# treangenlab/Seqwin

Measured on AMD Instinct MI355X. Metric: Gbp/s minimizer-indexed, higher is better.
Workload: dtype u64

## Files before the change

### seqwin_amd/csrc/radix.hip

```cpp
#include <algorithm>
#include <cstdlib>
#include <cstring>
#include <vector>
#include <map>
#include <mutex>

#include "device.hpp"

namespace sw {
namespace {

constexpr int RS_ITEMS = 16;
#ifdef SW_RS_STAMPS
__device__ unsigned long long *g_rs_stamps = nullptr;
#define RS_STAMP(i)                                                                                        \
    do {                                                                                                   \
        if (g_rs_stamps && (tile & 63u) == 0 && threadIdx.x == 0) g_rs_stamps[(size_t)(tile >> 6) * 16 + (i)] = clock64(); \
    } while (0)
#else
#define RS_STAMP(i) do { } while (0)
#endif
#ifndef RS_LOOK
#define RS_LOOK 4
#endif
// ... 920 lines not shown
            unsigned long long *ptr = stamps.p;
            SW_HIP(hipMemcpyToSymbolAsync(HIP_SYMBOL(g_rs_stamps), &ptr, sizeof ptr, 0, hipMemcpyHostToDevice, stream));
        }
#endif
        unsigned long long *cur = perm_hi32 && p == 0 ? cursor.p : nullptr;
        hipLaunchKernelGGL(k_rs_scan<BITS>, dim3(1), dim3(RADIX), 0, stream, hist.p + (size_t)p * RADIX, cur);
        const uint32_t epoch = cur ? 0u : next_epoch(su.b, stream);
        auto launch = [&](auto kern) {
            hipLaunchKernelGGL(kern, dim3((unsigned)std::min<uint64_t>(n_tiles, (uint64_t)grid_p)), dim3(THREADS), 0, stream, keys, alt, n,
                               (uint32_t)n_tiles, sh, bits, hist.p + (size_t)p * RADIX, su.b.p, tickets.p + p, d_fail, dbg, cur,
                               RS_CURSOR_STRIDE, 64u, epoch);
        };
        if (cur ? !ballot_forced() : atomic_rank) launch(k_rs_pass_p<THREADS, BITS, 1>);
        else launch(k_rs_pass_p<THREADS, BITS, 0>);
        SW_HIP(hipGetLastError());
#ifdef SW_RS_STAMPS
        if (stamps.p) {
            std::vector<unsigned long long> hs(n_st);
            SW_HIP(hipStreamSynchronize(stream));
            SW_HIP(hipMemcpy(hs.data(), stamps.p, stamps.bytes(), hipMemcpyDeviceToHost));
            double acc[8] = {0}, look[3] = {0};
            size_t cnt = 0;
            for (size_t t = 0; t + 16 <= n_st; t += 16) {
                if (!hs[t] || !hs[t + 7]) continue;
                for (int i = 1; i <= 7; ++i) acc[i] += (double)(hs[t + i] - hs[t + i - 1]);
                for (int i = 0; i < 3; ++i) look[i] += (double)hs[t + 8 + i];
                ++cnt;
            }
            static const char *nm[] = {"", "rank", "barrier", "totals+scan", "barrier+scatter", "lookback(d0)", "barrier", "write-out"};
            fprintf(stderr, "[rs stamps] %d x %d bits, pass %u, %zu tiles sampled; mean clocks:", THREADS, BITS, p, cnt);
            double sum = 0;
            for (int i = 1; i <= 7; ++i) { fprintf(stderr, " %s=%.0f", nm[i], cnt ? acc[i] / cnt : 0.0); sum += cnt ? acc[i] / cnt : 0.0; }
            fprintf(stderr, " | tile %.0f | look-back of digit 0: %.1f steps, %.1f polls of an unpublished record, %.1f records behind\n", sum,
                    cnt ? look[0] / cnt : 0.0, cnt ? look[1] / cnt : 0.0, cnt ? look[2] / cnt : 0.0);
        }
#endif
        std::swap(keys, alt);
    }
}

}

namespace {
__global__ void k_rs_perm_cursors(unsigned long long *__restrict__ cursor, uint32_t n_groups, uint32_t radix, uint32_t stride,
                                  unsigned group_bits, unsigned digit_shift)
{
    const uint32_t i = blockIdx.x * blockDim.x + threadIdx.x;
    if (i >= n_groups * radix) return;
    const uint64_t g = i / radix, d = i % radix;
    cursor[(size_t)i * stride] = (group_bits < 64 ? g << group_bits : 0ull) + (d << digit_shift);
}
}

bool radix_unsort_perm_begin(UnsortPerm &u, uint64_t n, unsigned low_bits, unsigned nbit, hipStream_t stream)
{
    constexpr int THREADS = 512, BITS = 8;
    constexpr uint32_t RADIX = 1u << BITS, TILE = THREADS * RS_ITEMS;
    static_assert(UNSORT_CURSOR_STRIDE == RS_CURSOR_STRIDE, "one cursor layout for the first pass and for a producer that scatters itself");
    if (n == 0 || nbit <= low_bits + 8 || nbit > low_bits + 16) return false;
    if ((1ull << (low_bits + 8)) % TILE) return false;
    u.low_bits = low_bits;
    u.hi_bits = nbit - low_bits - 8;
    u.n_groups = (uint32_t)((n + (1ull << (low_bits + 8)) - 1) >> (low_bits + 8));
    const uint64_t n_tiles = (n + TILE - 1) / TILE;
    u.n_tiles = (uint32_t)n_tiles;
    int dev = 0, per_cu = 0;
    SW_HIP(hipGetDevice(&dev));
    hipDeviceProp_t prop;
    SW_HIP(hipGetDeviceProperties(&prop, dev));
    SW_HIP(hipOccupancyMaxActiveBlocksPerMultiprocessor(&per_cu, k_rs_pass_p<THREADS, BITS, 0>, THREADS, 0));
    u.grid = (unsigned)std::min<uint64_t>(n_tiles, (uint64_t)std::max(1, per_cu) * std::max(1, prop.multiProcessorCount));
    if (!u.cur_a.p) {
        u.cur_a.alloc((size_t)RADIX * RS_CURSOR_STRIDE);
        u.cur_b.alloc((size_t)u.n_groups * RADIX);
        u.tickets.alloc(2);
    }
    SW_HIP(hipMemsetAsync(u.tickets.p, 0, 8, stream));
    hipLaunchKernelGGL(k_rs_perm_cursors, dim3(1), dim3(RADIX), 0, stream, u.cur_a.p, 1u, RADIX, RS_CURSOR_STRIDE, 64u, low_bits + 8);
    hipLaunchKernelGGL(k_rs_perm_cursors, dim3((u.n_groups * RADIX + 255) / 256), dim3(256), 0, stream, u.cur_b.p, u.n_groups, RADIX, 1u,
                       low_bits + 8, low_bits);
    SW_HIP(hipGetLastError());
    return true;
}

void radix_unsort_perm_first(UnsortPerm &u, const uint64_t *keys, uint64_t *alt, uint64_t n, hipStream_t stream, uint32_t *d_fail)
{
    constexpr int THREADS = 512, BITS = 8;
    auto pass = ballot_forced() ? k_rs_pass_p<THREADS, BITS, 0> : k_rs_pass_p<THREADS, BITS, 1>;
    hipLaunchKernelGGL(pass, dim3(u.grid), dim3(THREADS), 0, stream, keys, alt, n, u.n_tiles, 32u + u.low_bits + 8, u.hi_bits,
                       (const unsigned long long *)nullptr, (unsigned long long *)nullptr, u.tickets.p, d_fail, 0u, u.cur_a.p,
                       RS_CURSOR_STRIDE, 64u, 0u);
    SW_HIP(hipGetLastError());
}

void radix_unsort_perm_second(UnsortPerm &u, const uint64_t *keys, uint64_t *alt, uint64_t n, hipStream_t stream, uint32_t *d_fail)
{
    constexpr int THREADS = 512, BITS = 8;
    auto pass = ballot_forced() ? k_rs_pass_p<THREADS, BITS, 0> : k_rs_pass_p<THREADS, BITS, 1>;
    hipLaunchKernelGGL(pass, dim3(u.grid), dim3(THREADS), 0, stream, keys, alt, n, u.n_tiles, 32u + u.low_bits, 8u,
                       (const unsigned long long *)nullptr, (unsigned long long *)nullptr, u.tickets.p + 1, d_fail, 0u, u.cur_b.p, 1u,
                       u.low_bits + 8, 0u);
    SW_HIP(hipGetLastError());
}

bool radix_unsort_perm(uint64_t *&keys, uint64_t *&alt, uint64_t n, unsigned low_bits, unsigned nbit, hipStream_t stream, uint32_t *d_fail)
{
    UnsortPerm u;
    if (!radix_unsort_perm_begin(u, n, low_bits, nbit, stream)) return false;
    radix_unsort_perm_first(u, keys, alt, n, stream, d_fail);
    std::swap(keys, alt);
    radix_unsort_perm_second(u, keys, alt, n, stream, d_fail);
    std::swap(keys, alt);
    return true;
}

bool radix_pairs_available() { return rank_mode() == 1; }
int radix_rank_mode() { return rank_mode(); }

uint64_t radix_trim_state()
{
    uint64_t freed = 0;
    if (g_state_uses) return 0;
    std::lock_guard<std::mutex> lock(state_registry_mu());
    for (auto &kv : state_registry()) {
        StateBuf &b = *kv.second;
        std::unique_lock<std::mutex> use(b.mu, std::try_to_lock);
        if (!use.owns_lock() || !b.p) continue;
        int cur = -1;
        (void)hipGetDevice(&cur);
        if (cur != kv.first.first) (void)hipSetDevice(kv.first.first);
        (void)hipFree(b.p);
        if (cur != kv.first.first && cur >= 0) (void)hipSetDevice(cur);
        freed += b.words * 8;
        b.p = nullptr;
        b.words = 0;
        b.epoch = 0;
    }
    return freed;
}

void radix_demote_rank()
{
    int dev = 0;
    SW_HIP(hipGetDevice(&dev));
    std::lock_guard<std::mutex> lock(rank_mu());
    rank_modes()[dev] = 0;
}

void radix_sort_pairs32(uint32_t *&keys, uint32_t *&keys_alt, OccPay *&vals, OccPay *&vals_alt, uint64_t n, unsigned end_bit,
                        hipStream_t stream, uint32_t *d_fail, const StageSource *src, const std::function<void()> &after_first,
                        uint32_t *low_out)
{
    constexpr uint32_t RADIX = 1u << RP_BITS, TILE = RP_THREADS * RP_ITEMS;
    if (n == 0 || end_bit == 0) return;
    if (end_bit > 32 || end_bit % RP_BITS) raise(SW_ERR_RUNTIME, "radix_sort_pairs32: key bits must be a multiple of 8 up to 32");
    if (n >= 0xFFFFFFFFull) raise(SW_ERR_RUNTIME, "radix_sort_pairs32: more than 2^32-2 elements");
    const unsigned n_passes = end_bit / RP_BITS;
    const uint64_t n_tiles = (n + TILE - 1) / TILE;
    int grid_p = 0;
    {
        static std::mutex &mu = *new std::mutex;
        static std::map<int, int> &grids = *new std::map<int, int>;
        int dev = 0;
        SW_HIP(hipGetDevice(&dev));
        std::lock_guard<std::mutex> lock(mu);
        int &g = grids[dev];
        if (!g) {
            int per_cu = 0;
            hipDeviceProp_t prop;
            SW_HIP(hipGetDeviceProperties(&prop, dev));
            SW_HIP(hipOccupancyMaxActiveBlocksPerMultiprocessor(&per_cu, k_rs_pair_pass<0>, RP_THREADS, 0));
            g = std::max(1, per_cu) * std::max(1, prop.multiProcessorCount);
        }
        grid_p = g;
    }
    DevArray<unsigned long long> hist((size_t)n_passes * RADIX);
    DevArray<uint32_t> tickets(n_passes);
    SW_HIP(hipMemsetAsync(tickets.p, 0, tickets.bytes(), stream));
    SW_HIP(hipMemsetAsync(hist.p, 0, hist.bytes(), stream));
    StageSource stage{};
    DevArray<uint32_t> chunk_tile;
    DevArray<unsigned long long> chunk_dir;
    if (src && src->rows) {
        stage = *src;
        hipLaunchKernelGGL(k_rs_hist32_rows, dim3((unsigned)((n + 16383) / 16384)), dim3(256), 0, stream,
                           reinterpret_cast<const uint4 *>(src->rows), n, n_passes, hist.p);
    } else if (src) {
        constexpr uint64_t CHUNK = 64 * RP_ITEMS;
        static_assert(TILE == (RP_THREADS / 64) * CHUNK, "a tile is one chunk per wave");
        const uint64_t n_chunks = (n + CHUNK - 1) / CHUNK;
        stage = *src;
        chunk_tile.alloc(n_chunks);
        chunk_dir.alloc(n_chunks * STAGE_ROW);
        stage.chunk_dir = chunk_dir.p;
        hipLaunchKernelGGL(k_rs_chunk_tiles, dim3((stage.n_tiles + 255u) / 256u), dim3(256), 0, stream, stage.tile_count, stage.dst_off,
                           stage.n_tiles, chunk_tile.p);
        hipLaunchKernelGGL(k_rs_stage_prepare, dim3((unsigned)std::min<uint64_t>(2048, (n_chunks + 3) / 4)), dim3(256), 0, stream, stage,
                           (const uint32_t *)chunk_tile.p, n, n_passes, chunk_dir.p, hist.p);
    } else {
        hipLaunchKernelGGL(k_rs_hist32, dim3((unsigned)((n + 65535) / 65536)), dim3(256), 0, stream, keys, n, n_passes, hist.p);
    }
    SW_HIP(hipGetLastError());
    StateUse su = state_buf(stream, (size_t)n_tiles * RADIX);
    StateBuf &sb = su.b;
    const StageSource none{};
    const uint32_t fault = fault_rank();
    for (unsigned p = 0; p < n_passes; ++p) {
        hipLaunchKernelGGL(k_rs_scan<RP_BITS>, dim3(1), dim3(RADIX), 0, stream, hist.p + (size_t)p * RADIX, (unsigned long long *)nullptr);
        const uint32_t epoch = next_epoch(sb, stream);
        const dim3 grid((unsigned)std::min<uint64_t>(n_tiles, (uint64_t)grid_p));
        if (p == 0 && src) {
            auto first = src->rows ? k_rs_pair_pass<2> : k_rs_pair_pass<1>;
            hipLaunchKernelGGL(first, grid, dim3(RP_THREADS), 0, stream, (const uint32_t *)nullptr, (const uint4 *)nullptr,
                               keys_alt, reinterpret_cast<uint4 *>(vals_alt), n, (uint32_t)n_tiles, 0u,
                               (const unsigned long long *)hist.p, sb.p, epoch, tickets.p, d_fail, stage,
                               n_passes == 1 ? low_out : (uint32_t *)nullptr, fault);
            SW_HIP(hipGetLastError());
            if (after_first) after_first();
        } else {
            hipLaunchKernelGGL(k_rs_pair_pass<0>, grid, dim3(RP_THREADS), 0, stream, (const uint32_t *)keys,
                               reinterpret_cast<const uint4 *>(vals), keys_alt, reinterpret_cast<uint4 *>(vals_alt), n, (uint32_t)n_tiles,
                               RP_BITS * p, (const unsigned long long *)(hist.p + (size_t)p * RADIX), sb.p, epoch, tickets.p + p, d_fail,
                               none, p + 1 == n_passes ? low_out : (uint32_t *)nullptr, fault);
            SW_HIP(hipGetLastError());
        }
        std::swap(keys, keys_alt);
        std::swap(vals, vals_alt);
    }
}

namespace {
constexpr uint32_t EB_RADIX = 512, EB_TABLE = EB_RADIX * EB_RADIX, EB_THREADS = 512;
constexpr uint64_t EB_EMPTY = ~0ull;
static_assert(EB_THREADS == EB_RADIX, "k_eb_finish: one bin per thread");
enum : uint32_t { EB_F_OVERFLOW = 1u, EB_F_RANGE = 2u, EB_F_ORDER = 4u };
struct EbInfo {
    unsigned long long n_sentinels;
    uint32_t n_tiles2, max_bucket, flags, n_runs, n_live, pad;
};

__global__ __launch_bounds__(EB_RADIX) void k_eb_level1(const unsigned long long *__restrict__ h1, uint32_t tile_keys,
                                                        unsigned long long *__restrict__ cursor, unsigned long long *__restrict__ segtab,
                                                        EbInfo *__restrict__ info)
{
    __shared__ unsigned long long s[EB_RADIX];
    __shared__ uint32_t st[EB_RADIX];
    const uint32_t d = threadIdx.x;
    const unsigned long long c = h1[d];
    const uint32_t tiles = (uint32_t)((c + tile_keys - 1) / tile_keys);
    s[d] = c;
    st[d] = tiles;
    __syncthreads();
    for (uint32_t o = 1; o < EB_RADIX; o <<= 1) {
        const unsigned long long a = d >= o ? s[d - o] : 0;
        const uint32_t b = d >= o ? st[d - o] : 0;
        __syncthreads();
        s[d] += a;
        st[d] += b;
        __syncthreads();
    }
    const unsigned long long first = s[d] - c;
    cursor[(size_t)d * RS_CURSOR_STRIDE] = first;
    uint32_t w = st[d] - tiles;
    for (uint32_t t = 0; t < tiles; ++t)
        segtab[w + t] = seg_pack(first + (uint64_t)t * tile_keys, d, (uint32_t)min((unsigned long long)tile_keys, c - (uint64_t)t * tile_keys));
    if (d == EB_RADIX - 1) info->n_tiles2 = st[d];
}

__global__ __launch_bounds__(1024) void k_eb_count(const uint64_t *__restrict__ in, const unsigned long long *__restrict__ segtab,
                                                   const EbInfo *__restrict__ info, unsigned shift, uint32_t dmask, uint64_t sentinel,
                                                   uint32_t *__restrict__ table, EbInfo *__restrict__ out)
{
    __shared__ uint32_t hist[EB_RADIX];
    __shared__ uint32_t s_sent;
    const uint32_t n_tiles = info->n_tiles2;
    for (uint32_t w = blockIdx.x; w < n_tiles; w += gridDim.x) {
        const unsigned long long seg = segtab[w];
        const uint64_t first = seg_first(seg);
        const uint32_t cnt = seg_count(seg);
        if (threadIdx.x < EB_RADIX) hist[threadIdx.x] = 0;
        if (threadIdx.x == 0) s_sent = 0;
        __syncthreads();
        uint64_t key[RS_ITEMS];
#pragma unroll
        for (int i = 0; i < RS_ITEMS; ++i) {
            const uint32_t li = i * 1024 + threadIdx.x;
            key[i] = li < cnt ? in[first + li] : EB_EMPTY;
        }
        uint32_t sent = 0;
#pragma unroll
        for (int i = 0; i < RS_ITEMS; ++i) {
            if (key[i] == EB_EMPTY) continue;
            if (key[i] == sentinel) ++sent;
            atomicAdd(&hist[(uint32_t)(key[i] >> shift) & dmask], 1u);
        }
        if (sent) atomicAdd(&s_sent, sent);
        __syncthreads();
        if (threadIdx.x < EB_RADIX && hist[threadIdx.x]) atomicAdd(&table[seg_bucket(seg) * EB_RADIX + threadIdx.x], hist[threadIdx.x]);
        if (threadIdx.x == 0 && s_sent) atomicAdd(&out->n_sentinels, (unsigned long long)s_sent);
        __syncthreads();
    }
}

__global__ __launch_bounds__(1024) void k_eb_scan(const uint32_t *__restrict__ cnt, const unsigned long long *__restrict__ n_sent,
                                                  uint32_t sent_at, uint32_t *__restrict__ start, unsigned long long *__restrict__ cursor,
                                                  uint32_t *__restrict__ max_out, uint32_t *__restrict__ total_out,
                                                  uint4 *__restrict__ live, uint32_t *__restrict__ n_live_out)
{
    constexpr uint32_t PER4 = EB_TABLE / 1024 / 4;
    __shared__ uint32_t ws[16], wm[16], wz[16];
    const uint32_t tid = threadIdx.x, lane = tid & 63u, wave = tid >> 6;
    const uint32_t sent = n_sent ? (uint32_t)*n_sent : 0u;
    const uint4 *cnt4 = reinterpret_cast<const uint4 *>(cnt) + (size_t)tid * PER4;
    uint32_t sum = 0, mx = 0, nz = 0;
#pragma unroll 16
    for (uint32_t j = 0; j < PER4; ++j) {
        const uint4 c = cnt4[j];
        mx = max(max(max(mx, c.x), max(c.y, c.z)), c.w);
        sum += c.x + c.y + c.z + c.w;
        nz += (c.x != 0) + (c.y != 0) + (c.z != 0) + (c.w != 0);
    }
    if (n_sent && sent_at / (4 * PER4) == tid) {
        mx = 0;
        for (uint32_t j = 0; j < 4 * PER4; ++j) {
            const uint32_t i = tid * 4 * PER4 + j, c = cnt[i];
            mx = max(mx, c - (i == sent_at ? min(c, sent) : 0u));
        }
    }
    uint32_t incl = sum, inz = nz;
    for (uint32_t o = 1; o < 64; o <<= 1) {
        const uint32_t up = __shfl_up(incl, o, 64), uz = __shfl_up(inz, o, 64);
        if (lane >= o) {
            incl += up;
            inz += uz;
        }
        mx = max(mx, __shfl_xor(mx, o, 64));
    }
    if (lane == 63) {
        ws[wave] = incl;
        wz[wave] = inz;
    }
    if (lane == 0) wm[wave] = mx;
    __syncthreads();
    uint32_t run = incl - sum, below = inz - nz, n_live = 0;
    for (uint32_t w = 0; w < 16; ++w) {
        if (w < wave) {
            run += ws[w];
            below += wz[w];
        }
        n_live += wz[w];
    }
    uint32_t at = n_live - 1u - below;
    uint4 *start4 = reinterpret_cast<uint4 *>(start) + (size_t)tid * PER4;
    ulonglong2 *cur2 = reinterpret_cast<ulonglong2 *>(cursor) + (size_t)tid * PER4 * 2;
#pragma unroll 16
    for (uint32_t j = 0; j < PER4; ++j) {
        const uint4 c = cnt4[j];
        const uint4 st = make_uint4(run, run + c.x, run + c.x + c.y, run + c.x + c.y + c.z);
        start4[j] = st;
        if (cursor) {
            cur2[2 * j] = make_ulonglong2(st.x, st.y);
            cur2[2 * j + 1] = make_ulonglong2(st.z, st.w);
        }
        if (live) {
            const uint32_t id = (tid * PER4 + j) * 4;
            if (c.x) live[at--] = make_uint4(id, st.x, c.x, 0u);
            if (c.y) live[at--] = make_uint4(id + 1, st.y, c.y, 0u);
            if (c.z) live[at--] = make_uint4(id + 2, st.z, c.z, 0u);
            if (c.w) live[at--] = make_uint4(id + 3, st.w, c.w, 0u);
        }
        run = st.w + c.w;
    }
    if (tid == 1023) {
        start[EB_TABLE] = run;
        if (total_out) *total_out = run;
        if (n_live_out) *n_live_out = n_live;
        uint32_t m = 0;
        for (uint32_t w = 0; w < 16; ++w) m = max(m, wm[w]);
        if (max_out) *max_out = m;
    }
}

#ifdef SW_RS_STAMPS
__device__ unsigned long long *g_eb_stamps = nullptr;
constexpr uint32_t EB_ST_EVERY = 16, EB_ST_WORDS = 16;
#define EB_STAMP(i) do { if (st) st[i] = clock64(); } while (0)
#define EB_STAMP_ADD(i, since) do { if (st) { const unsigned long long t_ = clock64(); st[i] += t_ - (since); (since) = t_; } } while (0)
#else
#define EB_STAMP(i) do { } while (0)
#define EB_STAMP_ADD(i, since) do { } while (0)
#endif

template <bool PACKED>
__global__ __launch_bounds__(EB_THREADS) void k_eb_finish(const uint64_t *__restrict__ in, const uint4 *__restrict__ live, uint32_t slots,
                                                          unsigned shift1, unsigned shift2, uint32_t mask2, unsigned bin_shift,
                                                          uint32_t bin_mask, unsigned cb, uint64_t sentinel,
                                                          uint64_t *__restrict__ tk, uint32_t *__restrict__ tc,
                                                          uint32_t *__restrict__ n_distinct, uint32_t *__restrict__ flags)
{
    extern __shared__ __align__(16) unsigned char eb_lds[];
    unsigned long long *hk = reinterpret_cast<unsigned long long *>(eb_lds);
    uint32_t *hc = reinterpret_cast<uint32_t *>(hk + slots);
    uint16_t *idx = PACKED ? reinterpret_cast<uint16_t *>(hk + slots) : reinterpret_cast<uint16_t *>(hc + slots);
    __shared__ uint32_t bd[EB_RADIX + 1], bk[EB_RADIX], bcur[EB_RADIX], wsd[EB_THREADS / 64], wsk[EB_THREADS / 64];
    __shared__ uint32_t s_over;
    const uint32_t tid = threadIdx.x, lane = tid & 63u, wave = tid >> 6;
#ifdef SW_RS_STAMPS
    unsigned long long *st = g_eb_stamps && tid == 0 && blockIdx.x % EB_ST_EVERY == 0 ? g_eb_stamps + (size_t)(blockIdx.x / EB_ST_EVERY) * EB_ST_WORDS : nullptr;
    unsigned long long st_t = 0;
#endif
    EB_STAMP(0);
    const uint4 me = live[blockIdx.x];
    const uint32_t mask = slots - 1u;
    for (uint32_t s = tid; s < slots; s += EB_THREADS) {
        hk[s] = EB_EMPTY;
        if (!PACKED) hc[s] = 0;
    }
    bd[tid] = 0;
    bk[tid] = 0;
    if (tid == 0) s_over = 0;
    const uint32_t b = me.x, first = me.y, cnt = me.z;
    const uint64_t low_mask = (1ull << shift2) - 1ull, count_mask = (1ull << cb) - 1ull;
    const uint64_t high = ((uint64_t)(b / EB_RADIX) << shift1) | ((uint64_t)(b % EB_RADIX) << shift2);
    uint64_t nxt[4];
#pragma unroll
    for (int i = 0; i < 4; ++i) {
        const uint32_t j = i * EB_THREADS + tid;
        nxt[i] = j < cnt ? in[(uint64_t)first + j] : sentinel;
    }
    EB_STAMP(1);
    __syncthreads();
    EB_STAMP(2);
#ifdef SW_RS_STAMPS
    if (st) st_t = clock64();
#endif
    uint32_t bad = 0;
    for (uint32_t j0 = 0; j0 < cnt; j0 += 4 * EB_THREADS) {
        if (*(volatile uint32_t *)&s_over) break;
        uint64_t key[4];
#pragma unroll
        for (int i = 0; i < 4; ++i) key[i] = nxt[i];
        if (j0 + 4 * EB_THREADS < cnt) {
#pragma unroll
            for (int i = 0; i < 4; ++i) {
                const uint32_t j = j0 + 4 * EB_THREADS + i * EB_THREADS + tid;
                nxt[i] = j < cnt ? in[(uint64_t)first + j] : sentinel;
            }
        }
        uint32_t cp[4], h[4];
        unsigned long long w[4];
#pragma unroll
        for (int i = 0; i < 4; ++i) {
            const uint64_t k = key[i];
            bool alive = k != sentinel;
            if (alive && ((uint32_t)(k >> shift1) * EB_RADIX + ((uint32_t)(k >> shift2) & mask2)) != b) {
                bad = 1;
                alive = false;
            }
            uint32_t copies = 1;
            const uint64_t any = __ballot(alive);
            if (any) {
                const int src = __ffsll((long long)any) - 1;
                const uint64_t k0 = (uint64_t)__shfl((unsigned long long)k, src, 64);
                const uint64_t same = __ballot(alive && k == k0);
                if (alive && k == k0) {
                    copies = (uint32_t)__popcll(same);
                    alive = (int)lane == src;
                }
            }
            cp[i] = alive ? copies : 0u;
            h[i] = (uint32_t)((k * 0x9E3779B97F4A7C15ull) >> 40) & mask;
            w[i] = PACKED ? ((k & low_mask) << cb) | copies : (unsigned long long)k;
        }
        EB_STAMP_ADD(3, st_t);
        for (uint32_t probes = 0; cp[0] | cp[1] | cp[2] | cp[3]; ++probes) {
            if (probes == slots) {
                s_over = 1;
                break;
            }
            unsigned long long old[4];
#pragma unroll
            for (int i = 0; i < 4; ++i)
                if (cp[i]) old[i] = atomicCAS(&hk[h[i]], EB_EMPTY, w[i]);
#pragma unroll
            for (int i = 0; i < 4; ++i) {
                if (!cp[i]) continue;
                if (PACKED) {
                    if (old[i] == EB_EMPTY) cp[i] = 0;
                    else if ((old[i] >> cb) == (w[i] >> cb)) {
                        atomicAdd(&hk[h[i]], (unsigned long long)cp[i]);
                        cp[i] = 0;
                    } else h[i] = (h[i] + 1u) & mask;
                } else {
                    if (old[i] == EB_EMPTY || old[i] == w[i]) {
                        atomicAdd(&hc[h[i]], cp[i]);
                        cp[i] = 0;
                    } else h[i] = (h[i] + 1u) & mask;
                }
            }
        }
        EB_STAMP_ADD(4, st_t);
    }
    if (bad) atomicOr(flags, EB_F_RANGE);
    __syncthreads();
    EB_STAMP(5);
    if (s_over) {
        if (tid == 0) atomicOr(flags, EB_F_OVERFLOW);
        return;
    }
    const unsigned wbin_shift = PACKED ? bin_shift + cb : bin_shift;
    for (uint32_t s = tid; s < slots; s += EB_THREADS) {
        const uint64_t k = hk[s];
        if (k == EB_EMPTY) continue;
        const uint32_t bin = (uint32_t)(k >> wbin_shift) & bin_mask;
        atomicAdd(&bd[bin], 1u);
        atomicAdd(&bk[bin], PACKED ? (uint32_t)(k & count_mask) : hc[s]);
    }
    __syncthreads();
    EB_STAMP(6);
    {
        const uint32_t d = bd[tid], c = bk[tid];
        uint32_t id = d, ic = c;
        for (uint32_t o = 1; o < 64; o <<= 1) {
            const uint32_t ud = __shfl_up(id, o, 64), uc = __shfl_up(ic, o, 64);
            if (lane >= o) {
                id += ud;
                ic += uc;
            }
        }
        if (lane == 63) {
            wsd[wave] = id;
            wsk[wave] = ic;
        }
        __syncthreads();
        uint32_t pd = id - d, pc = ic - c;
        for (uint32_t w2 = 0; w2 < wave; ++w2) {
            pd += wsd[w2];
            pc += wsk[w2];
        }
        bd[tid] = pd;
        bcur[tid] = pd;
        bk[tid] = pc;
        if (tid == EB_THREADS - 1) bd[EB_RADIX] = pd + d;
    }
    __syncthreads();
    EB_STAMP(7);
    for (uint32_t s = tid; s < slots; s += EB_THREADS) {
        const uint64_t k = hk[s];
        if (k == EB_EMPTY) continue;
        idx[atomicAdd(&bcur[(uint32_t)(k >> wbin_shift) & bin_mask], 1u)] = (uint16_t)s;
    }
    __syncthreads();
    EB_STAMP(8);
    const uint32_t n_dist = bd[EB_RADIX];
    if (tid == 0) n_distinct[b] = n_dist;
    for (uint32_t j = tid; j < n_dist; j += EB_THREADS) {
        const uint32_t s = idx[j];
        const uint64_t k = hk[s];
        const uint32_t bin = (uint32_t)(k >> wbin_shift) & bin_mask, lo = bd[bin], hi = bd[bin + 1];
        uint32_t less = 0, copies_less = 0;
        for (uint32_t i = lo; i < hi; i += 4) {
            uint32_t s2[4];
            unsigned long long k2[4];
            uint32_t c2[4];
#pragma unroll
            for (int u = 0; u < 4; ++u) s2[u] = i + u < hi ? idx[i + u] : s;
#pragma unroll
            for (int u = 0; u < 4; ++u) {
                k2[u] = hk[s2[u]];
                c2[u] = PACKED ? 0u : hc[s2[u]];
            }
#pragma unroll
            for (int u = 0; u < 4; ++u) {
                if (PACKED ? (k2[u] >> cb) < (k >> cb) : k2[u] < k) {
                    ++less;
                    copies_less += PACKED ? (uint32_t)(k2[u] & count_mask) : c2[u];
                }
            }
        }
        tk[(uint64_t)first + lo + less] = PACKED ? high | (k >> cb) : k;
        tc[(uint64_t)first + lo + less] = first + bk[bin] + copies_less;
    }
#ifdef SW_RS_STAMPS
    if (st) {
        st[9] = clock64();
        st[10] = cnt;
        st[11] = n_dist;
    }
#endif
}

__global__ __launch_bounds__(256) void k_eb_compact(const uint64_t *__restrict__ tk, const uint32_t *__restrict__ tc,
                                                    const uint4 *__restrict__ live, uint32_t n_live, const uint32_t *__restrict__ start,
                                                    const uint32_t *__restrict__ dstart,
                                                    const unsigned long long *__restrict__ n_sentinels, uint64_t *__restrict__ ukeys,
                                                    uint32_t *__restrict__ ucnt, uint32_t *__restrict__ flags)
{
    if (blockIdx.x == 0 && threadIdx.x == 0) ucnt[dstart[EB_TABLE]] = start[EB_TABLE] - (uint32_t)*n_sentinels;
    if (blockIdx.x >= n_live) return;
    const uint4 me = live[blockIdx.x];
    const uint32_t b = me.x, d0 = dstart[b], n = dstart[b + 1] - d0;
    if (n == 0) return;
    const uint64_t first = me.y;
    const uint32_t end = me.y + me.z;
    uint32_t bad = 0;
    for (uint32_t j = threadIdx.x; j < n; j += 256) {
        const uint64_t k = tk[first + j];
        const uint32_t c = tc[first + j];
        if (j + 1 < n && (tk[first + j + 1] <= k || tc[first + j + 1] <= c)) bad = 1;
        if (c < first || c >= end) bad = 1;
        ukeys[d0 + j] = k;
        ucnt[d0 + j] = c;
    }
    if (bad) atomicOr(flags, EB_F_ORDER);
}
}

int radix_edge_buckets(uint64_t *&keys, uint64_t *&alt, uint64_t m, unsigned key_bits, uint64_t sentinel,
                       const unsigned long long *d_hist_top, uint32_t cap, uint32_t slots, uint64_t *ukeys, uint32_t *ucnt,
                       uint32_t *n_runs, hipStream_t stream, uint32_t *d_fail, bool debug)
{
    constexpr int THREADS = 1024, BITS = 9;
    constexpr uint32_t TILE = THREADS * RS_ITEMS;
    unsigned digit_bits = 0, n_passes = 0;
    radix_layout(key_bits, &digit_bits, &n_passes);
    if (n_passes < 2 || m >= (1ull << 32) - 1 || slots < 64 || slots > 8192 || (slots & (slots - 1))) return 1;
    const unsigned shift1 = (n_passes - 1) * digit_bits, bits1 = key_bits - shift1;
    const unsigned bits2 = std::min<unsigned>(BITS, shift1), shift2 = shift1 - bits2;
    const unsigned bin_bits = std::min<unsigned>(BITS, shift2), bin_shift = shift2 - bin_bits;
    const uint64_t n_tiles = (m + TILE - 1) / TILE, max_tiles2 = n_tiles + EB_RADIX;
    int dev = 0, per_cu = 0;
    SW_HIP(hipGetDevice(&dev));
    hipDeviceProp_t prop;
    SW_HIP(hipGetDeviceProperties(&prop, dev));
    SW_HIP(hipOccupancyMaxActiveBlocksPerMultiprocessor(&per_cu, k_rs_pass_p<THREADS, BITS, 0>, THREADS, 0));
    const unsigned cus = (unsigned)std::max(1, prop.multiProcessorCount);
    const unsigned grid = (unsigned)std::min<uint64_t>(n_tiles, (uint64_t)std::max(1, per_cu) * cus);

    DevArray<unsigned long long> h1(EB_RADIX), cur1((size_t)EB_RADIX * RS_CURSOR_STRIDE), cur2(EB_TABLE), segtab(max_tiles2);
    DevArray<uint32_t> table(EB_TABLE), start(EB_TABLE + 1), tickets(2), flags(1);
    DevArray<uint4> live(EB_TABLE);
    DevArray<EbInfo> info(1);
    SW_HIP(hipMemsetAsync(h1.p, 0, h1.bytes(), stream));
    SW_HIP(hipMemsetAsync(table.p, 0, table.bytes(), stream));
    SW_HIP(hipMemsetAsync(tickets.p, 0, 8, stream));
    SW_HIP(hipMemsetAsync(flags.p, 0, 4, stream));
    SW_HIP(hipMemsetAsync(info.p, 0, sizeof(EbInfo), stream));
    if (d_hist_top)
        SW_HIP(hipMemcpyAsync(h1.p, d_hist_top, (size_t)8 << digit_bits, hipMemcpyDeviceToDevice, stream));
    else
        hipLaunchKernelGGL(k_rs_hist<BITS>, dim3((unsigned)((m + 32767) / 32768)), dim3(256), 0, stream, (const uint64_t *)keys, m, shift1,
                           key_bits, 1u, h1.p);
    hipLaunchKernelGGL(k_eb_level1, dim3(1), dim3(EB_RADIX), 0, stream, (const unsigned long long *)h1.p, TILE, cur1.p, segtab.p, info.p);
    auto pass1 = ballot_forced() ? k_rs_pass_p<THREADS, BITS, 0> : k_rs_pass_p<THREADS, BITS, 1>;
    hipLaunchKernelGGL(pass1, dim3(grid), dim3(THREADS), 0, stream, (const uint64_t *)keys, alt, m, (uint32_t)n_tiles, shift1, bits1,
                       (const unsigned long long *)nullptr, (unsigned long long *)nullptr, tickets.p, d_fail, 0u, cur1.p, RS_CURSOR_STRIDE,
                       64u, 0u);
    std::swap(keys, alt);
    hipLaunchKernelGGL(k_eb_count, dim3((unsigned)std::min<uint64_t>(max_tiles2, (uint64_t)8 * cus)), dim3(1024), 0, stream,
                       (const uint64_t *)keys, (const unsigned long long *)segtab.p, (const EbInfo *)info.p, shift2, (1u << bits2) - 1u,
                       sentinel, table.p, info.p);
    const uint32_t sent_at = (uint32_t)(sentinel >> shift1) * EB_RADIX + ((uint32_t)(sentinel >> shift2) & ((1u << bits2) - 1u));
    hipLaunchKernelGGL(k_eb_scan, dim3(1), dim3(1024), 0, stream, (const uint32_t *)table.p, (const unsigned long long *)&info.p->n_sentinels,
                       sent_at, start.p, cur2.p, &info.p->max_bucket, (uint32_t *)nullptr, live.p, &info.p->n_live);
    SW_HIP(hipGetLastError());
    EbInfo hi;
    SW_HIP(hipMemcpyAsync(&hi, info.p, sizeof hi, hipMemcpyDeviceToHost, stream));
    SW_HIP(hipStreamSynchronize(stream));
    unsigned cb = 1;
    while (cb < 32 && (hi.max_bucket >> cb)) ++cb;
    const bool eligible = shift2 + cb <= 63;
    bool packed = eligible;
    if (const char *e = SW_TEST_GETENV("SEQWIN_AMD_EDGE_FINISH")) packed = !strcmp(e, "packed");
    const bool refused = packed && !eligible;
    const size_t lds = (size_t)slots * (packed ? 10 : 14);
    auto finish = packed ? k_eb_finish<true> : k_eb_finish<false>;
    static std::mutex &mu = *new std::mutex;
    static int lds_set[2] = {0, 0};
    {
        std::lock_guard<std::mutex> lock(mu);
        lds_set[packed] = std::max(lds_set[packed], (int)lds);
        SW_HIP(hipFuncSetAttribute(reinterpret_cast<const void *>(finish), hipFuncAttributeMaxDynamicSharedMemorySize, lds_set[packed]));
    }
    if (debug) {
        int resident = 0;
        SW_HIP(hipOccupancyMaxActiveBlocksPerMultiprocessor(&resident, finish, EB_THREADS, lds));
        fprintf(stderr, "[edge buckets] %llu keys, %llu sentinels, digits %u+%u+%u of %u bits, largest sub-bucket %u (capacity %u, %u slots)%s; "
                        "%u live sub-buckets, %s slots%s, %d workgroups per CU\n",
                (unsigned long long)m, hi.n_sentinels, bits1, bits2, bin_bits, key_bits, hi.max_bucket, cap, slots,
                hi.max_bucket > cap ? ": radix passes instead" : "", hi.n_live, packed ? "packed" : "plain",
                refused ? " do not fit: radix passes instead" : "", resident);
    }
    if (hi.max_bucket > cap || refused) return 1;
    auto pass2 = ballot_forced() ? k_rs_pass_p<THREADS, BITS, 0, true> : k_rs_pass_p<THREADS, BITS, 1, true>;
    hipLaunchKernelGGL(pass2, dim3(std::max(1u, std::min(hi.n_tiles2, (uint32_t)(std::max(1, per_cu) * cus)))), dim3(THREADS), 0, stream,
                       (const uint64_t *)keys, alt, m, hi.n_tiles2, shift2, bits2, (const unsigned long long *)segtab.p,
                       (unsigned long long *)nullptr, tickets.p + 1, d_fail, 0u, cur2.p, 1u, 64u, 0u);
    std::swap(keys, alt);
    DevArray<uint32_t> tc(m), n_distinct(EB_TABLE), dstart(EB_TABLE + 1);
    SW_HIP(hipMemsetAsync(n_distinct.p, 0, n_distinct.bytes(), stream));
    uint64_t *tk = alt;
#ifdef SW_RS_STAMPS
    DevArray<unsigned long long> stamps;
    const size_t n_st = (size_t)(hi.n_live / EB_ST_EVERY + 1) * EB_ST_WORDS;
    if (getenv("SEQWIN_AMD_STAMPS")) {
        stamps.alloc(n_st);
        SW_HIP(hipMemsetAsync(stamps.p, 0, stamps.bytes(), stream));
        unsigned long long *ptr = stamps.p;
        SW_HIP(hipMemcpyToSymbolAsync(HIP_SYMBOL(g_eb_stamps), &ptr, sizeof ptr, 0, hipMemcpyHostToDevice, stream));
    }
#endif
    if (hi.n_live)
        hipLaunchKernelGGL(finish, dim3(hi.n_live), dim3(EB_THREADS), lds, stream, (const uint64_t *)keys, (const uint4 *)live.p, slots, shift1,
                           shift2, (1u << bits2) - 1u, bin_shift, (1u << bin_bits) - 1u, cb, sentinel, tk, tc.p, n_distinct.p, flags.p);
#ifdef SW_RS_STAMPS
    if (stamps.p) {
        std::vector<unsigned long long> hs(n_st);
        SW_HIP(hipStreamSynchronize(stream));
        SW_HIP(hipMemcpy(hs.data(), stamps.p, stamps.bytes(), hipMemcpyDeviceToHost));
        unsigned long long *none = nullptr;
        SW_HIP(hipMemcpyToSymbol(HIP_SYMBOL(g_eb_stamps), &none, sizeof none));
        double acc[10] = {0}, keys_sum = 0, dist_sum = 0;
        size_t cnt = 0;
        for (size_t t = 0; t + EB_ST_WORDS <= n_st; t += EB_ST_WORDS) {
            if (!hs[t] || !hs[t + 9] || hs[t + 10] <= 2 * 4 * EB_THREADS || hs[t + 10] > 3 * 4 * EB_THREADS) continue;
            acc[1] += (double)(hs[t + 1] - hs[t]);
            acc[2] += (double)(hs[t + 2] - hs[t + 1]);
            acc[3] += (double)hs[t + 3];
            acc[4] += (double)hs[t + 4];
            acc[5] += (double)(hs[t + 5] - hs[t + 2]) - (double)hs[t + 3] - (double)hs[t + 4];
            for (int i = 6; i <= 9; ++i) acc[i] += (double)(hs[t + i] - hs[t + i - 1]);
            keys_sum += (double)hs[t + 10];
            dist_sum += (double)hs[t + 11];
            ++cnt;
        }
        static const char *nm[] = {"", "entry+list", "init+barrier", "merge(+key wait)", "probes", "loop barrier", "bin count", "scan", "scatter", "rank+store"};
        fprintf(stderr, "[eb stamps] %s slots, %zu workgroups of 3 steps sampled (mean %.0f keys, %.0f distinct); mean clocks:", packed ? "packed" : "plain",
                cnt, cnt ? keys_sum / cnt : 0.0, cnt ? dist_sum / cnt : 0.0);
        double sum = 0;
        for (int i = 1; i <= 9; ++i) { fprintf(stderr, " %s=%.0f", nm[i], cnt ? acc[i] / cnt : 0.0); sum += cnt ? acc[i] / cnt : 0.0; }
        fprintf(stderr, " | workgroup %.0f\n", sum);
    }
#endif
    hipLaunchKernelGGL(k_eb_scan, dim3(1), dim3(1024), 0, stream, (const uint32_t *)n_distinct.p, (const unsigned long long *)nullptr, 0u,
                       dstart.p, (unsigned long long *)nullptr, (uint32_t *)nullptr, &info.p->n_runs, (uint4 *)nullptr, (uint32_t *)nullptr);
    hipLaunchKernelGGL(k_eb_compact, dim3(std::max(1u, hi.n_live)), dim3(256), 0, stream, (const uint64_t *)tk, (const uint32_t *)tc.p,
                       (const uint4 *)live.p, hi.n_live, (const uint32_t *)start.p, (const uint32_t *)dstart.p,
                       (const unsigned long long *)&info.p->n_sentinels, ukeys, ucnt, flags.p);
    SW_HIP(hipGetLastError());
    uint32_t hf = 0;
    SW_HIP(hipMemcpyAsync(&hi, info.p, sizeof hi, hipMemcpyDeviceToHost, stream));
    SW_HIP(hipMemcpyAsync(&hf, flags.p, 4, hipMemcpyDeviceToHost, stream));
    SW_HIP(hipStreamSynchronize(stream));
    if (hf & (EB_F_RANGE | EB_F_ORDER))
        raise(SW_ERR_RUNTIME, "internal error: the edge buckets are out of order (%s)", hf & EB_F_RANGE ? "a key outside its bucket" : "run starts descend");
    if (hf & EB_F_OVERFLOW) {
        if (debug) fprintf(stderr, "[edge buckets] a sub-bucket holds more than %u distinct keys: radix passes instead\n", slots);
        return 1;
    }
    *n_runs = hi.n_runs;
    return 0;
}

static int pick_shape(unsigned bits)
{
    const char *e = SW_TEST_GETENV("SEQWIN_AMD_RADIX_BITS");
    const bool nine = e ? atoi(e) == 9 : (bits + 8) / 9 < (bits + 7) / 8;
    return nine ? 1 : 0;
}

void radix_layout(unsigned bits, unsigned *digit_bits, unsigned *n_passes)
{
    const int sh = pick_shape(bits);
    *digit_bits = sh == 1 ? 9u : 8u;
    *n_passes = (bits + *digit_bits - 1) / *digit_bits;
}

void radix_sort_keys64(uint64_t *&keys, uint64_t *&alt, uint64_t n, unsigned begin_bit, unsigned end_bit, hipStream_t stream,
                       uint32_t *d_fail, bool perm_hi32, unsigned long long *d_hist_given, unsigned layout_bits)
{
    if (n == 0 || end_bit <= begin_bit) return;
    if (end_bit - begin_bit > 64) raise(SW_ERR_RUNTIME, "radix_sort_keys64: more than 64 key bits");
    switch (pick_shape(layout_bits ? layout_bits : end_bit - begin_bit)) {
    case 1: sort_passes<1024, 9>(keys, alt, n, begin_bit, end_bit, stream, d_fail, perm_hi32, d_hist_given); break;
    default: sort_passes<512, 8>(keys, alt, n, begin_bit, end_bit, stream, d_fail, perm_hi32, d_hist_given); break;
    }
}

}
```

Before: 499.3.

## Split edge-bucket scan across workgroups and early-exit finish on global overflow

```diff
diff --git a/seqwin_amd/csrc/radix.hip b/seqwin_amd/csrc/radix.hip
--- a/seqwin_amd/csrc/radix.hip
+++ b/seqwin_amd/csrc/radix.hip
@@ -1246,6 +1246,8 @@
     }
 }
 
+constexpr uint32_t EB_SCAN_WGS = 16;
+static_assert(EB_TABLE / 1024 / 4 % EB_SCAN_WGS == 0, "k_eb_scan: a thread's 16-byte loads divide among the workgroups");
 __global__ __launch_bounds__(1024) void k_eb_scan(const uint32_t *__restrict__ cnt, const unsigned long long *__restrict__ n_sent,
                                                   uint32_t sent_at, uint32_t *__restrict__ start, unsigned long long *__restrict__ cursor,
                                                   uint32_t *__restrict__ max_out, uint32_t *__restrict__ total_out,
@@ -1256,9 +1258,14 @@
     const uint32_t tid = threadIdx.x, lane = tid & 63u, wave = tid >> 6;
     const uint32_t sent = n_sent ? (uint32_t)*n_sent : 0u;
     const uint4 *cnt4 = reinterpret_cast<const uint4 *>(cnt) + (size_t)tid * PER4;
-    uint32_t sum = 0, mx = 0, nz = 0;
+    const uint32_t j_lo = blockIdx.x * (PER4 / gridDim.x), j_hi = j_lo + PER4 / gridDim.x;
+    uint32_t sum = 0, mx = 0, nz = 0, sum_lo = 0, nz_lo = 0;
 #pragma unroll 16
     for (uint32_t j = 0; j < PER4; ++j) {
+        if (j == j_lo) {
+            sum_lo = sum;
+            nz_lo = nz;
+        }
         const uint4 c = cnt4[j];
         mx = max(max(max(mx, c.x), max(c.y, c.z)), c.w);
         sum += c.x + c.y + c.z + c.w;
@@ -1294,11 +1301,13 @@
         }
         n_live += wz[w];
     }
-    uint32_t at = n_live - 1u - below;
+    const uint32_t total = run + sum;
+    run += sum_lo;
+    uint32_t at = n_live - 1u - below - nz_lo;
     uint4 *start4 = reinterpret_cast<uint4 *>(start) + (size_t)tid * PER4;
     ulonglong2 *cur2 = reinterpret_cast<ulonglong2 *>(cursor) + (size_t)tid * PER4 * 2;
-#pragma unroll 16
-    for (uint32_t j = 0; j < PER4; ++j) {
+#pragma unroll 4
+    for (uint32_t j = j_lo; j < j_hi; ++j) {
         const uint4 c = cnt4[j];
         const uint4 st = make_uint4(run, run + c.x, run + c.x + c.y, run + c.x + c.y + c.z);
         start4[j] = st;
@@ -1315,9 +1324,9 @@
         }
         run = st.w + c.w;
     }
-    if (tid == 1023) {
-        start[EB_TABLE] = run;
-        if (total_out) *total_out = run;
+    if (tid == 1023 && blockIdx.x == 0) {
+        start[EB_TABLE] = total;
+        if (total_out) *total_out = total;
         if (n_live_out) *n_live_out = n_live;
         uint32_t m = 0;
         for (uint32_t w = 0; w < 16; ++w) m = max(m, wm[w]);
@@ -1354,15 +1363,24 @@
     unsigned long long st_t = 0;
 #endif
     EB_STAMP(0);
+    uint32_t &s_seen = bcur[0];
     const uint4 me = live[blockIdx.x];
+    uint32_t fl = 0;
+    if (lane == 0) fl = __hip_atomic_load(flags, __ATOMIC_RELAXED, __HIP_MEMORY_SCOPE_AGENT);
+    const bool gone = (__builtin_amdgcn_readfirstlane(fl) & EB_F_OVERFLOW) != 0;
     const uint32_t mask = slots - 1u;
-    for (uint32_t s = tid; s < slots; s += EB_THREADS) {
-        hk[s] = EB_EMPTY;
-        if (!PACKED) hc[s] = 0;
-    }
-    bd[tid] = 0;
-    bk[tid] = 0;
-    if (tid == 0) s_over = 0;
+    if (!gone) {
+        for (uint32_t s = tid; s < slots; s += EB_THREADS) {
+            hk[s] = EB_EMPTY;
+            if (!PACKED) hc[s] = 0;
+        }
+        bd[tid] = 0;
+        bk[tid] = 0;
+    }
+    if (tid == 0) {
+        s_over = 0;
+        s_seen = 0;
+    }
     const uint32_t b = me.x, first = me.y, cnt = me.z;
     const uint64_t low_mask = (1ull << shift2) - 1ull, count_mask = (1ull << cb) - 1ull;
     const uint64_t high = ((uint64_t)(b / EB_RADIX) << shift1) | ((uint64_t)(b % EB_RADIX) << shift2);
@@ -1370,7 +1388,7 @@
 #pragma unroll
     for (int i = 0; i < 4; ++i) {
         const uint32_t j = i * EB_THREADS + tid;
-        nxt[i] = j < cnt ? in[(uint64_t)first + j] : sentinel;
+        nxt[i] = !gone && j < cnt ? in[(uint64_t)first + j] : sentinel;
     }
     EB_STAMP(1);
     __syncthreads();
@@ -1378,9 +1396,14 @@
 #ifdef SW_RS_STAMPS
     if (st) st_t = clock64();
 #endif
+    if (gone) s_seen = 1;
     uint32_t bad = 0;
-    for (uint32_t j0 = 0; j0 < cnt; j0 += 4 * EB_THREADS) {
-        if (*(volatile uint32_t *)&s_over) break;
+    for (uint32_t j0 = 0; !gone && j0 < cnt; j0 += 4 * EB_THREADS) {
+        if (__builtin_amdgcn_readfirstlane(fl) & EB_F_OVERFLOW) {
+            s_seen = 1;
+            break;
+        }
+        if (*(volatile uint32_t *)&s_over | *(volatile uint32_t *)&s_seen) break;
         uint64_t key[4];
 #pragma unroll
         for (int i = 0; i < 4; ++i) key[i] = nxt[i];
@@ -1390,6 +1413,7 @@
                 const uint32_t j = j0 + 4 * EB_THREADS + i * EB_THREADS + tid;
                 nxt[i] = j < cnt ? in[(uint64_t)first + j] : sentinel;
             }
+            if (lane == 0) fl = __hip_atomic_load(flags, __ATOMIC_RELAXED, __HIP_MEMORY_SCOPE_AGENT);
         }
         uint32_t cp[4], h[4];
         unsigned long long w[4];
@@ -1448,8 +1472,8 @@
     if (bad) atomicOr(flags, EB_F_RANGE);
     __syncthreads();
     EB_STAMP(5);
-    if (s_over) {
-        if (tid == 0) atomicOr(flags, EB_F_OVERFLOW);
+    if (s_over | s_seen) {
+        if (tid == 0 && s_over) atomicOr(flags, EB_F_OVERFLOW);
         return;
     }
     const unsigned wbin_shift = PACKED ? bin_shift + cb : bin_shift;
@@ -1605,7 +1629,7 @@
                        (const uint64_t *)keys, (const unsigned long long *)segtab.p, (const EbInfo *)info.p, shift2, (1u << bits2) - 1u,
                        sentinel, table.p, info.p);
     const uint32_t sent_at = (uint32_t)(sentinel >> shift1) * EB_RADIX + ((uint32_t)(sentinel >> shift2) & ((1u << bits2) - 1u));
-    hipLaunchKernelGGL(k_eb_scan, dim3(1), dim3(1024), 0, stream, (const uint32_t *)table.p, (const unsigned long long *)&info.p->n_sentinels,
+    hipLaunchKernelGGL(k_eb_scan, dim3(EB_SCAN_WGS), dim3(1024), 0, stream, (const uint32_t *)table.p, (const unsigned long long *)&info.p->n_sentinels,
                        sent_at, start.p, cur2.p, &info.p->max_bucket, (uint32_t *)nullptr, live.p, &info.p->n_live);
     SW_HIP(hipGetLastError());
     EbInfo hi;
@@ -1686,7 +1710,7 @@
         fprintf(stderr, " | workgroup %.0f\n", sum);
     }
 #endif
-    hipLaunchKernelGGL(k_eb_scan, dim3(1), dim3(1024), 0, stream, (const uint32_t *)n_distinct.p, (const unsigned long long *)nullptr, 0u,
+    hipLaunchKernelGGL(k_eb_scan, dim3(EB_SCAN_WGS), dim3(1024), 0, stream, (const uint32_t *)n_distinct.p, (const unsigned long long *)nullptr, 0u,
                        dstart.p, (unsigned long long *)nullptr, (uint32_t *)nullptr, &info.p->n_runs, (uint4 *)nullptr, (uint32_t *)nullptr);
     hipLaunchKernelGGL(k_eb_compact, dim3(std::max(1u, hi.n_live)), dim3(256), 0, stream, (const uint64_t *)tk, (const uint32_t *)tc.p,
                        (const uint4 *)live.p, hi.n_live, (const uint32_t *)start.p, (const uint32_t *)dstart.p,
```

After: 497.8. No clear change (-0.3%).
